# liaojing/videomorphing

Measured on AMD Instinct MI355X. Metric: Mpixel*iters/s (halfway optimizer, 1080p pair, 6-level pyramid, 500 iters/level), higher is better.
Workload: dtype f32

## Files before the change

include/vmorph.h:

```cpp
#ifndef VMORPH_H
#define VMORPH_H

#include <stdint.h>

#ifdef __cplusplus
extern "C" {
#endif

#define VM_OK            0
#define VM_E_INVALID    -1
#define VM_E_DEVICE     -2
#define VM_E_STATE      -3
#define VM_E_NUMERIC    -4
#define VM_E_CANCELLED  -5

typedef struct vm_ctx vm_ctx;
typedef struct vm_pyr vm_pyr;

enum { VM_BCOND_NONE = 0, VM_BCOND_CORNER = 1, VM_BCOND_BORDER = 2 };

typedef struct {
    float w_temp, w_ui, w_tps, w_ssim;
    float ssim_clamp;
    float eps;
// ... 29 lines not shown
    int    iters_live;
    double clk_shader_ticks[2];
    double clk_wall_ticks[2];
} vm_progress;

enum {
    VM_F_IMG0 = 0, VM_F_IMG1, VM_F_V, VM_F_LUMA, VM_F_MEAN, VM_F_VAR, VM_F_CROSS,
    VM_F_VALUE, VM_F_COUNTER, VM_F_TPS_AXY, VM_F_TPS_B, VM_F_UI_AXY, VM_F_UI_B,
    VM_F_IMPMASK,
    VM_F_TEMP_REF, VM_F_TEMP_MASK, VM_F_FLOW_F0, VM_F_FLOW_F1, VM_F_FLOW_B0, VM_F_FLOW_B1
};

const char *vm_last_error(void);
const char *vm_version(void);

int  vm_ctx_create(int device, vm_ctx **out);
void vm_ctx_destroy(vm_ctx *ctx);
int  vm_ctx_sync(vm_ctx *ctx);
int  vm_set_params(vm_ctx *ctx, const vm_kern_params *p);
int  vm_get_params(vm_ctx *ctx, vm_kern_params *p);
int  vm_set_math_mode(vm_ctx *ctx, int mode);
enum { VM_SWEEP_AUTO = 0, VM_SWEEP_TILE = 1, VM_SWEEP_SPLIT = 2, VM_SWEEP_STEP = 3, VM_SWEEP_SPARSE = 4, VM_SWEEP_PASS = 5 };
int  vm_set_tuning(vm_ctx *ctx, int sweep_mode, int threads, int parts);
int  vm_set_commit_order(vm_ctx *ctx, int order);
#define VM_REDUCE_ATOMIC 0
#define VM_REDUCE_ORDERED 1
int  vm_set_reduction(vm_ctx *ctx, int mode);
int  vm_dbg_pass_force_timeout(vm_ctx *ctx, int on);
int  vm_dbg_pass_fallbacks(vm_ctx *ctx);
int  vm_dbg_sparse_resident(vm_ctx *ctx, int mode);
int  vm_dbg_sparse_resident_visits(vm_ctx *ctx);
int  vm_dbg_pass_placement(vm_ctx *ctx, uint8_t *xcc_of_block, int n);
int  vm_dbg_golden(vm_ctx *ctx, int n, const float *params, float eps, uint32_t *out);
int  vm_dbg_streams_overlap(vm_ctx *a, vm_ctx *b, int *overlap);
int  vm_dbg_pyramid_scale(vm_ctx *ctx, const float *planes, int w, int h, int wout, int hout, float *out);
int  vm_device_info(vm_ctx *ctx, char *name256, int *cus, uint64_t *hbm_bytes);

int  vm_pyramid_create(vm_ctx *ctx, int nlevels, const int *w, const int *h, vm_pyr **out);
void vm_pyramid_destroy(vm_pyr *pyr);
int  vm_pyramid_levels(vm_pyr *pyr);
int  vm_level_dims(vm_pyr *pyr, int lvl, int *w, int *h, int *rowstride);
int  vm_level_upload_luma(vm_pyr *pyr, int lvl, const float *img0, const float *img1, int pitch);
int  vm_pyramid_build_rgb(vm_pyr *pyr, const uint8_t *rgb0, const uint8_t *rgb1, int pitch_bytes);
int  vm_level_set_v(vm_pyr *pyr, int lvl, const float *v_xy, int pitch);
int  vm_level_get_v(vm_pyr *pyr, int lvl, float *v_xy, int pitch);
int  vm_level_get_field(vm_pyr *pyr, int lvl, int field, void *host);
int  vm_level_clear(vm_pyr *pyr, int lvl);
int  vm_dbg_level_set_mask(vm_pyr *pyr, int lvl, const uint32_t *words);

int  vm_coarse_solve(vm_pyr *pyr, int lvl, int w0, int h0, const vm_constraint *c, int n);
int  vm_upsample_v(vm_pyr *pyr, int dst_lvl, int src_lvl);
int  vm_init_level(vm_pyr *pyr, int lvl, int w0, int h0, const vm_constraint *c, int n);
int  vm_optimize_level(vm_pyr *pyr, int lvl, float max_iter, volatile const int *run_flag,
                       int fixed_work, vm_progress *out);
int  vm_solve(vm_pyr *pyr, float max_iter, float max_iter_drop_factor,
              const vm_constraint *c, int n, volatile const int *run_flag,
              int fixed_work, vm_progress *per_level);
int  vm_optimize_level_batch(vm_pyr **pyrs, int n, int lvl, float max_iter,
                             volatile const int *run_flag, int fixed_work, vm_progress *out);
int  vm_solve_batch(vm_pyr **pyrs, int n, float max_iter, float max_iter_drop_factor,
                    volatile const int *run_flag, int fixed_work, vm_progress *per_level);
int  vm_solve_batch_cons(vm_pyr **pyrs, int n, float max_iter, float max_iter_drop_factor,
                         const vm_constraint *const *cons, const int *ncons,
                         volatile const int *run_flag, int fixed_work, vm_progress *per_level);
int  vm_upscale_result(vm_pyr *pyr, int lvl, int w0, int h0, float *v_xy_out, int pitch);

// ... 241 lines not shown
```

videomorphing_amd/capi.py:

```python
import ctypes as C
import os

_HERE = os.path.dirname(os.path.abspath(__file__))
LIB_PATH = os.environ.get("VM_LIB_PATH") or os.path.join(_HERE, "lib", "libvmorph_hip.so")

VM_OK = 0
VM_E_INVALID, VM_E_DEVICE, VM_E_STATE, VM_E_NUMERIC, VM_E_CANCELLED = -1, -2, -3, -4, -5
BCOND_NONE, BCOND_CORNER, BCOND_BORDER = 0, 1, 2
MATH_EXACT, MATH_FAST, MATH_EXACT_FMA, MATH_REF_FASTMATH, MATH_REF_TEX8, MATH_REF_TEX8_TRUNC = 0, 1, 2, 3, 4, 5
REDUCE_ATOMIC, REDUCE_ORDERED = 0, 1
DBG_MGB_QPATH = 3
SWEEP_AUTO, SWEEP_TILE, SWEEP_SPLIT, SWEEP_STEP, SWEEP_SPARSE, SWEEP_PASS = 0, 1, 2, 3, 4, 5
ERR_SSIM, ERR_TPS, ERR_UI, ERR_TEMP, ERR_ALL = 0, 1, 2, 3, 4
ERR_NAMES = ("ssim", "tps", "ui", "temp", "all")
EASE_LINEAR, EASE_SMOOTH = 0, 1
FILTER_BILINEAR, FILTER_CATMULL_ROM, FILTER_MITCHELL, FILTER_BSPLINE = 0, 1, 2, 3

FIELDS = {
    "img0": (0, 1), "img1": (1, 1), "v": (2, 2), "luma": (3, 2), "mean": (4, 2), "var": (5, 2),
    "cross": (6, 1), "value": (7, 1), "counter": (8, 1), "tps_axy": (9, 1), "tps_b": (10, 2),
    "ui_axy": (11, 1), "ui_b": (12, 2), "impmask": (13, 1),
    "temp_ref": (14, 2), "temp_mask": (15, 1), "f0": (16, 2), "f1": (17, 2), "b0": (18, 2), "b1": (19, 2),
}

SYMBOLS = [
    "vm_last_error", "vm_version", "vm_ctx_create", "vm_ctx_destroy", "vm_ctx_sync",
    "vm_set_params", "vm_get_params", "vm_set_math_mode", "vm_set_tuning", "vm_set_commit_order", "vm_set_reduction", "vm_dbg_pass_placement", "vm_dbg_pass_force_timeout",
    "vm_dbg_pass_fallbacks", "vm_dbg_golden", "vm_dbg_level_set_mask", "vm_dbg_sparse_resident", "vm_dbg_sparse_resident_visits", "vm_dbg_streams_overlap", "vm_dbg_pyramid_scale", "vm_device_info",
    "vm_pyramid_create", "vm_pyramid_destroy", "vm_pyramid_levels", "vm_level_dims",
    "vm_level_upload_luma", "vm_pyramid_build_rgb", "vm_level_set_v", "vm_level_get_v", "vm_level_get_field",
    "vm_level_clear", "vm_coarse_solve", "vm_upsample_v", "vm_init_level", "vm_optimize_level",
    "vm_solve", "vm_optimize_level_batch", "vm_solve_batch", "vm_solve_batch_cons", "vm_upscale_result", "vm_frame_create", "vm_frame_destroy", "vm_frame_upload", "vm_frame_upload_rgb",
    "vm_frame_download_ext", "vm_host_register", "vm_host_unregister", "vm_frame_set_v_from_level", "vm_render_halfway",
    "vm_render_halfway_dev", "vm_poisson_extend", "vm_poisson_extend_frames", "vm_frame_quadratic_path", "vm_frame_download_qpath", "vm_frame_download_v",
    "vm_rccl_bcast", "vm_rccl_comm_init_all", "vm_rccl_comm_destroy", "vm_bcast_params", "vm_bcast_bytes", "vm_dbg_poisson_profile",
    "vm_dbg_mgb_setup", "vm_dbg_mgb_level", "vm_dbg_mgb_cycle",
    "vm_video_create", "vm_video_destroy", "vm_video_levels", "vm_video_level_dims", "vm_video_upload_luma",
    "vm_video_upload_flows", "vm_video_build_rgb", "vm_video_build_flows", "vm_video_set_v", "vm_video_get_v",
    "vm_video_get_field", "vm_video_coarse_solve", "vm_video_upsample", "vm_video_init_level",
    "vm_video_initialize_temp", "vm_video_optimize_level", "vm_video_solve", "vm_video_result", "vm_frame_set_v_from_video",
    "vm_sync_level_table", "vm_sync_create", "vm_sync_destroy", "vm_sync_set_constraints", "vm_sync_load_identity",
    "vm_sync_upsample_level", "vm_sync_optimize_level", "vm_sync_solve", "vm_sync_get_field", "vm_sync_set_field",
    "vm_sync_result", "vm_sync_upload_frame", "vm_sync_upload_flow", "vm_sync_render", "vm_sync_render_dev",
    "vm_flow_params_default", "vm_optical_flow_rgb", "vm_optical_flow_luma", "vm_video_build_flows_rgb", "vm_sync_compute_flows",
    "vm_track_create", "vm_track_destroy", "vm_track_upload_frame", "vm_track_upload_flows", "vm_track_compute_flows",
    "vm_track_get_flows", "vm_track_propagate", "vm_video_build_flows_track",
    "vm_level_energy", "vm_level_energy_batch", "vm_level_error_map", "vm_level_error_image",
    "vm_video_energy", "vm_video_error_map", "vm_video_error_image",
    "vm_frame_sampling_maps", "vm_frame_upload_layers", "vm_render_layers", "vm_render_layers_dev",
    "vm_frame_upload_schedule", "vm_frame_clear_schedule", "vm_render_transition", "vm_render_transition_dev",
    "vm_render_transition_layers", "vm_render_transition_layers_dev", "vm_frame_transition_maps",
    "vm_render_shutter", "vm_render_shutter_dev", "vm_render_shutter_layers", "vm_render_shutter_layers_dev",
    "vm_render_transition_shutter", "vm_render_transition_shutter_dev", "vm_render_transition_shutter_layers",
    "vm_render_transition_shutter_layers_dev",
    "vm_render_viewport", "vm_render_viewport_dev", "vm_render_viewport_layers", "vm_render_viewport_layers_dev",
    "vm_frame_render_viewport_filtered", "vm_frame_render_viewport_filtered_dev", "vm_frame_render_viewport_filtered_layers",
    "vm_frame_render_viewport_filtered_layers_dev",
    "vm_render_viewport_shutter", "vm_render_viewport_shutter_dev", "vm_render_viewport_shutter_layers",
    "vm_render_viewport_shutter_layers_dev",
    "vm_render_viewport_transition_shutter", "vm_render_viewport_transition_shutter_dev",
    "vm_render_viewport_transition_shutter_layers", "vm_render_viewport_transition_shutter_layers_dev",
# ... 63 lines not shown
class VmError(RuntimeError):
    def __init__(self, code, msg):
        RuntimeError.__init__(self, "vmorph error %d: %s" % (code, msg))
        self.code = code


_lib = None


def load():
    global _lib
    if _lib is not None:
        return _lib
    if not os.path.exists(LIB_PATH):
        raise ImportError("%s is missing: run `python -m videomorphing_amd.build` "
                          "(or __graft_entry__.build()); there is no fallback path" % LIB_PATH)
    L = C.CDLL(LIB_PATH)
    vp, i, f = C.c_void_p, C.c_int, C.c_float
    L.vm_last_error.restype = C.c_char_p
    L.vm_version.restype = C.c_char_p
    sig = {
        "vm_ctx_create": [i, C.POINTER(vp)],
        "vm_ctx_sync": [vp],
        "vm_set_params": [vp, C.POINTER(KernParams)],
        "vm_get_params": [vp, C.POINTER(KernParams)],
        "vm_set_math_mode": [vp, i],
        "vm_set_tuning": [vp, i, i, i],
        "vm_set_commit_order": [vp, i],
        "vm_set_reduction": [vp, i],
        "vm_dbg_pass_placement": [vp, vp, i],
        "vm_dbg_pass_force_timeout": [vp, i],
        "vm_dbg_pass_fallbacks": [vp],
        "vm_dbg_golden": [vp, i, vp, C.c_float, vp],
        "vm_dbg_sparse_resident": [vp, C.c_int],
        "vm_dbg_sparse_resident_visits": [vp],
        "vm_device_info": [vp, C.c_char_p, C.POINTER(i), C.POINTER(C.c_uint64)],
        "vm_pyramid_create": [vp, i, C.POINTER(i), C.POINTER(i), C.POINTER(vp)],
        "vm_pyramid_levels": [vp],
        "vm_level_dims": [vp, i, C.POINTER(i), C.POINTER(i), C.POINTER(i)],
        "vm_level_upload_luma": [vp, i, vp, vp, i],
        "vm_pyramid_build_rgb": [vp, vp, vp, i],
        "vm_level_set_v": [vp, i, vp, i],
        "vm_level_get_v": [vp, i, vp, i],
        "vm_level_get_field": [vp, i, i, vp],
        "vm_level_clear": [vp, i],
        "vm_dbg_level_set_mask": [vp, i, vp],
        "vm_coarse_solve": [vp, i, i, i, vp, i],
        "vm_upsample_v": [vp, i, i],
        "vm_init_level": [vp, i, i, i, vp, i],
        "vm_optimize_level": [vp, i, f, vp, i, C.POINTER(Progress)],
        "vm_solve": [vp, f, f, vp, i, vp, i, vp],
        "vm_optimize_level_batch": [vp, i, i, f, vp, i, vp],
        "vm_solve_batch": [vp, i, f, f, vp, i, vp],
        "vm_solve_batch_cons": [vp, i, f, f, vp, vp, vp, i, vp],
        "vm_upscale_result": [vp, i, i, i, vp, i],
        "vm_frame_create": [vp, i, i, i, C.POINTER(vp)],
        "vm_frame_upload": [vp, vp, vp, vp, vp],
        "vm_frame_upload_rgb": [vp, vp, vp, i],
        "vm_dbg_streams_overlap": [vp, vp, C.POINTER(i)],
        "vm_dbg_pyramid_scale": [vp, vp, i, i, i, i, vp],
        "vm_frame_download_ext": [vp, i, vp],
        "vm_frame_set_v_from_level": [vp, vp, i],
        "vm_render_halfway": [vp, f, f, i, vp, i],
        "vm_render_halfway_dev": [vp, f, f, i, C.POINTER(f)],
        "vm_poisson_extend": [vp, i, f, i, C.POINTER(i), C.POINTER(f), C.POINTER(f)],
        "vm_poisson_extend_frames": [C.POINTER(vp), i, f, i, C.POINTER(i), C.POINTER(f), C.POINTER(f)],
# ... 126 lines not shown
```

videomorphing_amd/csrc/vm_api.cpp:

```cpp
#include "vm_internal.h"
#include "vm_host.h"

#include <algorithm>
#include <cstdarg>
#include <cstdio>
#include <cstdlib>
#include <cstring>
#include <string>
#include <vector>

static thread_local std::string g_err;

int vm_fail(int code, const char *fmt, ...)
{
    char buf[512];
    va_list ap;
    va_start(ap, fmt);
    vsnprintf(buf, sizeof(buf), fmt, ap);
    va_end(ap);
    g_err = buf;
    return code;
}

extern "C" const char *vm_last_error(void) { return g_err.c_str(); }
// ... 217 lines not shown
        memset(xcc_of_block, 0xFF, (size_t)n);
        return VM_OK;
    }
    std::vector<uint32_t> h(2048);
    VM_HIP(hipStreamSynchronize(c->stream));
    VM_HIP(hipMemcpy(h.data(), c->pass_dbg.get(), 2048 * sizeof(uint32_t), hipMemcpyDeviceToHost));
    for (int k = 0; k < n; ++k) xcc_of_block[k] = (uint8_t)(h[k] & 0xFFu);
    return VM_OK;
}

extern "C" int vm_dbg_golden(vm_ctx *c, int n, const float *params, float eps, uint32_t *out)
{
    if (!params || !out || n < 1 || n > 65536) return vm_fail(VM_E_INVALID, "vm_dbg_golden: bad argument");
    if (!(eps >= 1.0f / 1024.0f && eps <= 1.0f)) return vm_fail(VM_E_INVALID, "vm_dbg_golden: eps %g (2^-10 to 1)", (double)eps);
    for (int k = 0; k < n; ++k)
        if (!(params[4 * k] >= 0.0f && params[4 * k] <= 16.0f))
            return vm_fail(VM_E_INVALID, "vm_dbg_golden: cc of case %d is %g (0 to 16)", k, (double)params[4 * k]);
    VM_ENTER_LOCKED(c);
    VmDev<float> in;
    VmDev<uint32_t> res;
    const size_t words = (size_t)n * VM_DBG_GOLDEN_WORDS;
    if (int rc = in.reserve((size_t)4 * n)) return rc;
    if (int rc = res.reserve(words)) return rc;
    hipStream_t s = c->stream;
    VM_HIP(hipMemcpyAsync(in.get(), params, (size_t)4 * n * sizeof(float), hipMemcpyHostToDevice, s));
    VM_HIP(hipMemsetAsync(res.get(), 0, words * sizeof(uint32_t), s));
    vm_launch_dbg_golden_fast(n, in.get(), eps, res.get(), s);
    VM_HIP(hipGetLastError());
    VM_HIP(hipMemcpyAsync(out, res.get(), words * sizeof(uint32_t), hipMemcpyDeviceToHost, s));
    VM_HIP(hipStreamSynchronize(s));
    return VM_OK;
}

extern "C" int vm_set_tuning(vm_ctx *c, int sweep_mode, int threads, int parts)
{
    if (!c || sweep_mode < VM_SWEEP_AUTO || sweep_mode > VM_SWEEP_PASS || threads < 0 || parts < 0 ||
        (threads && (threads % 64 || threads < 256 || threads > 1024)) || parts > 64)
        return vm_fail(VM_E_INVALID, "vm_set_tuning: bad argument");
    c->sweep_mode = sweep_mode;
    c->sweep_threads = threads;
    c->sweep_parts = parts;
    return VM_OK;
}

extern "C" int vm_device_info(vm_ctx *c, char *name256, int *cus, uint64_t *hbm)
{
    VM_ENTER(c);
    hipDeviceProp_t pr;
    VM_HIP(hipGetDeviceProperties(&pr, c->device));
    if (name256) snprintf(name256, 256, "%s (%s)", pr.name, pr.gcnArchName);
    if (cus) *cus = pr.multiProcessorCount;
    if (hbm) *hbm = (uint64_t)pr.totalGlobalMem;
    return VM_OK;
}

int vm_level_alloc(vm_ctx *c, vm_level &l, bool with_images)
{
    size_t n = (size_t)l.rs * l.h;
    size_t off = 0;
    size_t o_v = off; off += vm_align256(n * 8);
    size_t o_img0 = off, o_img1 = off, o_luma = off, o_mean = off, o_var = off, o_tpsb = off,
           o_uib = off, o_cross = off, o_value = off, o_uiaxy = off, o_imp = off;
    if (with_images) {
        o_img0 = off; off += vm_align256(n * 4);
        o_img1 = off; off += vm_align256(n * 4);
        o_luma = off; off += vm_align256(n * 8);
// ... 394 lines not shown
```

videomorphing_amd/csrc/vm_internal.h:

```cpp
#ifndef VM_INTERNAL_H
#define VM_INTERNAL_H

#include <hip/hip_runtime.h>
#include <stdint.h>
#include "../../include/vmorph.h"

#define VM_TILE_W 64
#define VM_TILE_H 16
#define VM_PITCH_X 69
#define VM_PITCH_Y 21
#define VM_HALO_W (VM_TILE_W + 4)
#define VM_HALO_H (VM_TILE_H + 4)
#define VM_NCELL (VM_HALO_W * VM_HALO_H)

struct VmLevelView {
    int w, h, rs;
    float inv_wh;
    int imp_rs, imp_rows;
    const float *img0, *img1;
    float2 *v, *luma, *mean, *var, *tps_b, *ui_b;
    float *cross, *value, *ui_axy;
    uint32_t *impmask;
    uint32_t *rec_tag;
    float4 *rec_a, *rec_b;
// ... 44 lines not shown
                                           uint32_t *stats, int iter_idx, int fixed_work,     \
                                           int threads, int parts, hipStream_t s);            \
    void vm_launch_optimize_step_##SUFFIX(const VmLevelView *views, int nbatch, int cap, int w,  \
                                          int h, const VmKParams &P, const uint32_t *tables,  \
                                          int offx, int offy, int pi, int pj, uint32_t epoch, \
                                          uint32_t prev_epoch, int src, int decide,           \
                                          uint32_t *flags, uint32_t *stats, int iter_idx,     \
                                          int fixed_work, int threads, int parts,             \
                                          uint32_t *slots_cur, const uint32_t *slots_prev,    \
                                          int prev_iter_idx, hipStream_t s);                  \
    void vm_launch_optimize_pass_##SUFFIX(const VmLevelView *views, int nbatch, int cap, int w,  \
                                          int h, const VmKParams &P, const uint32_t *tables,  \
                                          int offx, int offy, uint32_t epoch0, uint32_t *bar, \
                                          uint32_t *flags, uint32_t *stats, int iter_idx,     \
                                          int fixed_work, uint32_t *slots_cur,                \
                                          const uint32_t *slots_prev, int prev_iter_idx,      \
                                          uint32_t *err, uint32_t *dbg, int decide,           \
                                          int force_wt, hipStream_t s);                       \
    int vm_pass_resident_blocks_##SUFFIX(int device);                                         \
    void vm_launch_upsample_##SUFFIX(float2 *dst, int dw, int dh, int drs, const float2 *src, \
                                     int sw, int sh, int srs, hipStream_t s);                 \
    void vm_launch_splat_##SUFFIX(const VmLevelView &L, int w0, int h0,                       \
                                  const vm_constraint *dev_c, int n, hipStream_t s);

VM_DECL_LAUNCHERS(exact)
VM_DECL_LAUNCHERS(fast)
VM_DECL_LAUNCHERS(exactf)
VM_DECL_LAUNCHERS(reffm)
VM_DECL_LAUNCHERS(tex8)
VM_DECL_LAUNCHERS(tex8t)

#define VM_DBG_GOLDEN_WORDS 20
void vm_launch_dbg_golden_fast(int n, const float *in, float eps, uint32_t *out, hipStream_t s);

void vm_launch_upscale(float2 *dst, int w0, int h0, int dpitch, const float2 *v, int w, int h,
                       int rs, hipStream_t s);
void vm_launch_blend_v(float2 *dst, int dpitch, const float2 *a, const float2 *b, int spitch, int w0, int h0,
                       float alpha, float beta, hipStream_t s);
void vm_launch_render(uint8_t *out, int out_pitch, int w, int h, int rs, int ex, float color_fa,
                      float geo_fa, int color_from, const uchar4 *ext0, const uchar4 *ext1,
                      const float2 *v, const float2 *u, hipStream_t s);

#endif
```

videomorphing_amd/csrc/vm_sweep_kernels.hip:

```cpp
#include <algorithm>
#include <type_traits>
#include "vm_morph_common.h"

typedef __attribute__((address_space(1))) const uint32_t vm_g_cu32;
typedef __attribute__((address_space(1))) uint32_t vm_g_u32;
typedef __attribute__((address_space(1))) const unsigned long long vm_g_cu64;
typedef __attribute__((address_space(1))) unsigned long long vm_g_u64;
typedef __attribute__((address_space(1))) const float vm_g_cf32;

__device__ __forceinline__ int mad24(int a, int b, int c) { return __mul24(a, b) + c; }

namespace {

__device__ __forceinline__ int tile_cols(int w) { return (w + VM_PITCH_X - 1) / VM_PITCH_X; }
__device__ __forceinline__ int tile_rows(int h) { return (h + VM_PITCH_Y - 1) / VM_PITCH_Y; }
__device__ __forceinline__ int tile_ox(int t, int gx, int offx) { return (t % gx) * VM_PITCH_X + offx; }
__device__ __forceinline__ int tile_oy(int t, int gx, int offy) { return (t / gx) * VM_PITCH_Y + offy; }
__device__ __forceinline__ int phase_px(int ox, int slot, int pj) { return ox + (slot & 31) * 2 + pj; }
__device__ __forceinline__ int phase_py(int oy, int slot, int pi) { return oy + (slot >> 5) * 2 + pi; }
__device__ __forceinline__ void stage_imp(uint32_t *imp, const uint32_t *tables, int tid, int T) { for (int k = tid; k < 225; k += T) imp[k] = tables[VM_TAB_IMP + k]; }
__device__ __forceinline__ void stage_tps(float *tps, const uint32_t *tables, int tid, int T) { for (int k = tid; k < 625; k += T) tps[k] = __uint_as_float(tables[VM_TAB_TPS + k]); }
__device__ __forceinline__ float cell_count(int qy, int h, int qx, int w) { return (float)(window_count(qy, h) * window_count(qx, w)); }
__device__ __forceinline__ int window_row(int k) { return (k * 13) >> 6; }

// ... 691 lines not shown
    fj = __builtin_amdgcn_fmed3f(fj, -1.0f, (float)L.h);
    const int i = clamp0(L.w - 1, (int)fi + t.cx), j = clamp0(L.h - 1, (int)fj + t.cy);
    wgt = fmaf(t.wxs, a, t.wxo) * fmaf(t.wys, b, t.wyo);
    return (uint32_t)(t.imgoff + j * L.rs + i) << 2;
}
__device__ __forceinline__ void taps32_issue(const VmLevelView &L, const TapLane &t, const PixelCtx &c, float vx,
                                             float vy, float &texel, float &wgt)
{
    texel = *(vm_g_cf32 *)((const char *)L.img0 + taps32_addr(L, t, c, vx, vy, wgt));
}
struct TexelKeep {
    uint32_t off = 0xFFFFFFFFu;
    float texel = 0.0f;
};
__device__ __forceinline__ void taps32_issue(const VmLevelView &L, const TapLane &t, const PixelCtx &c, float vx,
                                             float vy, TexelKeep &keep, float &texel, float &wgt)
{
    const uint32_t off = taps32_addr(L, t, c, vx, vy, wgt);
    if (off != keep.off) {
        keep.texel = *(vm_g_cf32 *)((const char *)L.img0 + off);
        keep.off = off;
    }
    texel = keep.texel;
}
__device__ __forceinline__ void taps32_finish(const TapLane &t, float texel, float wgt, float &lx, float &ly)
{
    float r = texel * wgt;
    r += dpp_xor1(r);
    r += dpp_xor2(r);
    const float o = dpp_half_mirror(r);
    lx = t.odd ? o : r;
    ly = t.odd ? r : o;
}
__device__ __forceinline__ void taps32(const VmLevelView &L, const TapLane &t, const PixelCtx &c, float vx, float vy,
                                       TexelKeep &keep, float &lx, float &ly)
{
    float texel, wgt;
    taps32_issue(L, t, c, vx, vy, keep, texel, wgt);
    taps32_finish(t, texel, wgt, lx, ly);
}
__device__ __forceinline__ void line_lumas(const VmLevelView &L, const TapLane &t, const PixelCtx &c, float gx, float gy,
                                           float tmin, TexelKeep &keep, float2 &luma)
{
    taps32(L, t, c, fmaf(gx, tmin, c.v.x), fmaf(gy, tmin, c.v.y), keep, luma.x, luma.y);
}

template <bool INTERIOR>
__device__ __forceinline__ float change32(const VmKParams &P, const Nb1 &nb, const PixelCtx &c, float lx, float ly)
{
    const float dmx = lx - c.old_luma.x, dmy = ly - c.old_luma.y;
    const float dvx = lx * lx - c.old_luma.x * c.old_luma.x;
    const float dvy = ly * ly - c.old_luma.y * c.old_luma.y;
    const float dcross = lx * ly - c.old_luma.x * c.old_luma.y;
    float acc;
    if (INTERIOR) {
        const float val = ssim_core(window_mean(nb.A, dmx, 0.04f), window_mean(nb.B, dmy, 0.04f), nb.VX + dvx, nb.VY + dvy,
                                    nb.X + dcross, 25.0f, P.ssim_clamp);
        acc = nb.N != 0.0f ? nb.VAL - val : 0.0f;
    } else {
        const bool valid = nb.N != 0.0f;
        const float n = valid ? nb.N : 25.0f;
        const float in = n == 25.0f ? 0.04f : __builtin_amdgcn_rcpf(n);
        const float val = ssim_core(window_mean(nb.A, dmx, in), window_mean(nb.B, dmy, in), nb.VX + dvx, nb.VY + dvy,
                                    nb.X + dcross, n, P.ssim_clamp);
        acc = valid ? nb.VAL - val : 0.0f;
    }
// ... 89 lines not shown
    }
    const float R = 0.618033989f, C = 1.0f - R;
    float a = 0;
    float b = cc * C, x = b * R + cc * C;
    float fb, fx;
    ELINE(b, fb);
    ELINE(x, fx);
#pragma unroll 1
    for (;;) {
        if (!(cc - a > P.eps))
            break;
        const bool lt = fx < fb;
        const float p = lt ? x : b, qv = lt ? cc : a;
        a = lt ? b : a;
        cc = lt ? cc : x;
        const float xn = p * R + qv * C;
        float f;
        ELINE(xn, f);
        const float ob = b, ofb = fb;
        b = lt ? x : xn;
        x = lt ? xn : ob;
        fb = lt ? fx : f;
        fx = lt ? f : ofb;
    }
#undef ELINE
    const float tmin = fx < fb ? x : b, fmin = fx < fb ? fx : fb;
    if (!(fmin < 0))
        return false;
    step = make_float2(gx * tmin, gy * tmin);
    line_lumas(L, tl, c, gx, gy, tmin, keep, luma);
    return true;
}

#define GOLDEN64_NO_TRACE(T_)
#define GOLDEN64(EVAL2_, TRACE_, CC_, EPS_, HI_, NEVAL_, TMIN_, FMIN_)                                                 \
    {                                                                                                                  \
        const float R = 0.618033989f, C = 1.0f - R;                                                                    \
        float a = 0;                                                                                                   \
        float b = (CC_) * C, x = b * R + (CC_) * C;                                                                    \
        float fb, fx;                                                                                                  \
        EVAL2_((HI_) ? x : b, fb, fx);                                                                                 \
        TRACE_(b)                                                                                                      \
        TRACE_(x)                                                                                                      \
        (NEVAL_) += 2;                                                                                                 \
        _Pragma("unroll 1") while ((CC_) > (EPS_) && !(fx < fb))                                                       \
        {                                                                                                              \
            const float xn = b * R, xn2 = xn * R;                                                                      \
            float f1, f2;                                                                                              \
            EVAL2_((HI_) ? xn2 : xn, f1, f2);                                                                          \
            TRACE_(xn)                                                                                                 \
              \
            const bool held = x > (EPS_) && !(fb < f1);                                                                \
            if (held) {                       \
                TRACE_(xn2)                                                                                            \
            }                                                                                                          \
            (NEVAL_) += held ? 2 : 1;                                                                                  \
            (CC_) = held ? b : x;                                                                                      \
            x = held ? xn : b;                                                                                         \
            b = held ? xn2 : xn;                                                                                       \
            fx = held ? f1 : fb;                                                                                       \
            fb = held ? f2 : f1;                                                                                       \
        }                                                                                                              \
        _Pragma("unroll 1") for (;;)                                                                                   \
        {                                                                                                              \
            if (!((CC_) - a > (EPS_)))                                                                                 \
                break;                                                                                                 \
            const bool lt = fx < fb;                                                                                   \
                          \
            const float p = lt ? x : b, qv = lt ? (CC_) : a;                                                           \
            const float a1 = lt ? b : a, cc1 = lt ? (CC_) : x;                                                         \
            const float xn = p * R + qv * C;                                                                           \
            const float b1 = lt ? x : xn, x1 = lt ? xn : b;                                                            \
             \
               \
                      \
                                                                               \
            const bool G = lt;                                                                                         \
            const float p2 = G ? x1 : b1, q2 = G ? cc1 : a1;                                                           \
            const float xn2 = p2 * R + q2 * C;                                                                         \
            float f1, f2;                                                                                              \
            EVAL2_((HI_) ? xn2 : xn, f1, f2);                                                                          \
            TRACE_(xn)                                                                                                 \
            ++(NEVAL_);                                                                                                \
            {                                                                                                          \
                const float nfb = lt ? fx : f1, nfx = lt ? f1 : fb;                                                    \
                a = a1;                                                                                                \
                (CC_) = cc1;                                                                                           \
                b = b1;                                                                                                \
                x = x1;                                                                                                \
                fb = nfb;                                                                                              \
                fx = nfx;                                                                                              \
            }                                                                                                          \
            if ((CC_) - a > (EPS_) && (fx < fb) == G) {          \
                TRACE_(xn2)                                                                                            \
                const float ob = b, ofb = fb;                                                                          \
                a = G ? b : a;                                                                                         \
                (CC_) = G ? (CC_) : x;                                                                                 \
                b = G ? x : xn2;                                                                                       \
                x = G ? xn2 : ob;                                                                                      \
                fb = G ? fx : f2;                                                                                      \
                fx = G ? f2 : ofb;                                                                                     \
                ++(NEVAL_);                                                                                            \
            }                                                                                                          \
        }                                                                                                              \
        (TMIN_) = fx < fb ? x : b;                                                                                     \
        (FMIN_) = fx < fb ? fx : fb;                                                                                   \
    }

template <bool INTERIOR, class Ring>
__device__ __forceinline__ bool decide64(const VmLevelView &L, const VmKParams &P, const Nb1 &nb, const Ring &ring,
                                         const PixelCtx &c, int sub, bool hi, float2 &step, float2 &luma,
                                         uint32_t &n_eval)
{
    n_eval += 4;
    const bool has_temp = L.temp_mask != nullptr;
    const float WT = has_temp ? P.w_temp * c.tmask * L.factor_d * L.inv_wh : 0.0f;
    const TapLane tl = tap_lane_make(L, sub);
    float lx, ly;
    float gx = 0, gy = 0;
    {
        const float sgn = hi ? -1.0f : 1.0f;
        float g_tex[2], g_wgt[2];
#pragma unroll
        for (int r = 0; r < 2; ++r) {
            const float dx = r == 0 ? sgn * P.eps : 0.0f, dy = r == 0 ? 0.0f : sgn * P.eps;
            taps32_issue(L, tl, c, c.v.x + dx, c.v.y + dy, g_tex[r], g_wgt[r]);
        }
#pragma unroll
        for (int r = 0; r < 2; ++r) {
            const float dx = r == 0 ? sgn * P.eps : 0.0f, dy = r == 0 ? 0.0f : sgn * P.eps;
            taps32_finish(tl, g_tex[r], g_wgt[r], lx, ly);
            const float change = change32<INTERIOR>(P, nb, c, lx, ly);
            const float dd = dx * dx + dy * dy;
            const float v_tps = fmaf(c.tps_axy, dd, fmaf(c.tps_b.x, dx, c.tps_b.y * dy));
            const float v_ui = fmaf(c.ui_axy, dd, fmaf(c.ui_b.x, dx, c.ui_b.y * dy));
            float e = (P.w_ui * v_ui + P.w_ssim * change) * L.inv_wh + P.w_tps * v_tps;
            if (has_temp)
                e = fmaf(WT, temp_change(c, dx, dy), e);
            e *= sgn;
            float e_lo, e_hi;
            halves(e, e_lo, e_hi);
            if (r == 0) {
                gx += e_lo;
                gx += e_hi;
            } else {
                gy += e_lo;
                gy += e_hi;
            }
        }
    }
    gx = -gx;
    gy = -gy;
    const float ng = fsqrt(gx * gx + gy * gy);
    if (ng == 0)
        return false;
    gx = fdiv(gx, ng);
    gy = fdiv(gy, ng);
    float cc = fmaxf(fover32(L, ring, c, gx, gy, sub) - P.eps, 0.0f);
    const float gg = gx * gx + gy * gy;
    const float WS = P.w_ssim * L.inv_wh, WU = P.w_ui * L.inv_wh;
    const float Q2 = (WU * c.ui_axy + P.w_tps * c.tps_axy) * gg;
    const float Q1 = WU * (c.ui_b.x * gx + c.ui_b.y * gy) + P.w_tps * (c.tps_b.x * gx + c.tps_b.y * gy);
    const float T0 = fabsf(c.v.x - c.tref.x) + fabsf(c.v.y - c.tref.y);
    TexelKeep keep;
#define ELINE2(T_, FLO_, FHI_)                                                         \
    {                                                                                  \
        const float nvx_ = fmaf(gx, (T_), c.v.x), nvy_ = fmaf(gy, (T_), c.v.y);        \
        taps32(L, tl, c, nvx_, nvy_, keep, lx, ly);                                    \
        float f_ = fmaf(WS, change32<INTERIOR>(P, nb, c, lx, ly), (T_) * fmaf(Q2, (T_), Q1)); \
        if (has_temp)                                                                  \
            f_ = fmaf(WT, (fabsf(nvx_ - c.tref.x) + fabsf(nvy_ - c.tref.y)) - T0, f_); \
        halves(f_, (FLO_), (FHI_));                                                    \
    }
    float tmin, fmin;
    GOLDEN64(ELINE2, GOLDEN64_NO_TRACE, cc, P.eps, hi, n_eval, tmin, fmin)
#undef ELINE2
    if (!(fmin < 0))
        return false;
    step = make_float2(gx * tmin, gy * tmin);
    line_lumas(L, tl, c, gx, gy, tmin, keep, luma);
    return true;
}
#endif

__device__ __forceinline__ void ctx_load(PixelCtx &c, const VmLevelView &L, const float *s_tps, int px, int py)
{
    c.px = px;
    c.py = py;
    c.idx = py * L.rs + px;
    c.v = L.v[c.idx];
    c.old_luma = L.luma[c.idx];
    c.ui_axy = L.ui_axy[c.idx];
    c.ui_b = L.ui_b[c.idx];
    c.tps_axy = s_tps[(border_class(py, L.h) * 5 + border_class(px, L.w)) * 25 + 12] / 2;
    c.tref = make_float2(0, 0);
    c.tmask = 0.0f;
    if (L.temp_mask) {
        c.tref = L.temp_ref[c.idx];
        c.tmask = L.temp_mask[c.idx];
    }
}

__device__ __forceinline__ bool is_interior(const VmLevelView &L, int px, int py)
{
    return px >= 4 && px < L.w - 4 && py >= 4 && py < L.h - 4;
}

struct MaskGeom {
    int bx0, by0, nbx, nby;
// ... 282 lines not shown
                    hit = true;
                    cand = !pixel_locked(L, P.bcond, px, py);
                }
                S.d_ok[tid] = state;
            }
            bool any_hit;
            const int n_act = compact256(cand, tid, S.list, S.wave_cnt, hit, &any_hit);
            if (!any_hit)
                continue;

            if (n_act > 0) {
                st_cand += n_act;
#if !VM_EXACT
                if (!DENSE || (SMAX > 7 && INTV && n_act * 32 <= T)) {
                    const bool wide = n_act * 64 <= T;
                    for (int base = 0; base < n_act; base += wide ? T / 64 : T / 32) {
                    const int li = base + (wide ? tid >> 6 : tid >> 5), sub = tid & 31;
                    const bool writer = wide ? (tid & 63) == 0 : sub == 0;
                    const int slot = S.list[min(li, n_act - 1)];
                    const int tx = slot & 31, ty = slot >> 5;
                    const int px = ox + tx * 2 + pj, py = oy + ty * 2 + pi;
                    const bool wave_interior = __all(li >= n_act || is_interior(L, px, py));
                    if (li < n_act) {
                        PixelCtx c;
                        ctx_load(c, L, S.tps, px, py);
                        LdsSrc src{&S, (ty * 2 + pi) * VM_HALO_W + (tx * 2 + pj)};
                        c.tps_b = S.tpsb[src.hc + 2 * VM_HALO_W + 2];
                        float2 step = make_float2(0, 0), luma = make_float2(0, 0);
                        Nb1 nb;
                        bool ok;
                        uint32_t n_eval = 0;
                        if (wave_interior) {
                            nb1_load<true>(nb, L, src, c, sub);
                            ok = wide ? decide64<true>(L, P, nb, RingGlobal{L.v}, c, sub, (tid & 32) != 0, step, luma, n_eval)
                                      : decide32<true>(L, P, nb, RingGlobal{L.v}, c, sub, step, luma, n_eval);
                        } else {
                            nb1_load<false>(nb, L, src, c, sub);
                            ok = wide ? decide64<false>(L, P, nb, RingGlobal{L.v}, c, sub, (tid & 32) != 0, step, luma, n_eval)
                                      : decide32<false>(L, P, nb, RingGlobal{L.v}, c, sub, step, luma, n_eval);
                        }
                        if (writer)
                            atomicAdd(&S.n_eval, n_eval);
                        if (ok && writer) {
                            S.d_step[slot] = step;
                            S.d_mean[slot] = commit_dmean(luma, c.old_luma);
                            S.d_var[slot] = commit_dvar(luma, c.old_luma);
                            S.d_cross[slot] = commit_dcross(luma.x, luma.y, c.old_luma.x, c.old_luma.y);
                            L.luma[c.idx] = luma;
                            L.ui_b[c.idx] = commit_ui_b(c.ui_b, c.ui_axy, step);
                            L.v[c.idx] = commit_v(c.v, step);
                            S.d_ok[slot] = 3;
                        }
                    }
                    }
                } else
#else
                if (n_act * 32 <= 4 * T) {
                    const bool wide = n_act * 64 <= T;
                    for (int base = 0; base < n_act; base += wide ? T / 64 : T / 32) {
                        const int li = base + (wide ? tid >> 6 : tid >> 5), sub = tid & 31;
                        const bool writer = wide ? (tid & 63) == 0 : sub == 0;
                        const int slot = S.list[min(li, n_act - 1)];
                        const int tx = slot & 31, ty = slot >> 5;
                        const int px = ox + tx * 2 + pj, py = oy + ty * 2 + pi;
                        if (li < n_act) {
                            PixelCtx c;
                            ctx_load(c, L, S.tps, px, py);
                            LdsSrc src{&S, (ty * 2 + pi) * VM_HALO_W + (tx * 2 + pj)};
                            c.tps_b = S.tpsb[src.hc + 2 * VM_HALO_W + 2];
                            float2 step;
                            uint32_t n_eval = 0;
// ... 2140 lines not shown
                                                        int prev_iter_idx, int nslot_prev, int ntiles, int ngroups, int cap, int spread)
{
    pass_sum_slots(stats, slots_prev, prev_iter_idx, nslot_prev, ntiles, ngroups, cap, (int)threadIdx.x, spread != 0);
}

__global__ void SUF(k_next_iter)(int *iter_dev, int set, int value)
{
    if (threadIdx.x == 0 && blockIdx.x == 0)
        *iter_dev = set ? value : *iter_dev + value;
}

#if !VM_EXACT
__global__ __launch_bounds__(64) void SUF(k_dbg_golden)(const float *__restrict__ in, float eps, uint32_t *__restrict__ out)
{
    const int k = (int)blockIdx.x;
    const bool hi = (threadIdx.x & 32) != 0;
    float cc = in[4 * k];
    const float A = in[4 * k + 1], t0 = in[4 * k + 2], B = in[4 * k + 3];
    uint32_t *o = out + (size_t)k * VM_DBG_GOLDEN_WORDS;
    uint32_t n_eval = 0;
    int n_pt = 0;
#define EGOLDEN(T_, FLO_, FHI_)                     \
    {                                               \
        const float d_ = (T_) - t0;                 \
        const float f_ = (A * d_) * d_ + B;         \
        halves(f_, (FLO_), (FHI_));                 \
    }
#define TGOLDEN(T_)                                             \
    {                                                           \
        if (threadIdx.x == 0 && n_pt < VM_DBG_GOLDEN_WORDS - 3) \
            o[3 + n_pt] = __float_as_uint(T_);                  \
        ++n_pt;                                                 \
    }
    float tmin, fmin;
    GOLDEN64(EGOLDEN, TGOLDEN, cc, eps, hi, n_eval, tmin, fmin)
#undef EGOLDEN
#undef TGOLDEN
    if (threadIdx.x == 0) {
        o[0] = __float_as_uint(tmin);
        o[1] = __float_as_uint(fmin);
        o[2] = n_eval;
    }
}
#endif

}

void SUF(vm_launch_optimize)(const VmLevelView *views, int nbatch, int cap, int w, int h, const VmKParams &P,
                             const uint32_t *tables, int offx, int offy, uint32_t *flags, uint32_t *stats,
                             int iter_idx, int fixed_work, int threads, const int *iter_dev, int dense,
                             uint32_t *tile_list, hipStream_t s)
{
    dim3 b(threads), g((w + VM_PITCH_X - 1) / VM_PITCH_X, (h + VM_PITCH_Y - 1) / VM_PITCH_Y, nbatch);
#if !VM_EXACT
    if (!dense && tile_list) {
        const int nwords = ((w + 4) / 5 + 2) * ((h + 4) / 5 + 2), tiles = (int)(g.x * g.y);
        hipLaunchKernelGGL(SUF(k_tile_scan), dim3(std::min((nwords + 255) / 256, 32), 1, nbatch), dim3(256), 0, s, views, cap, offx,
                           offy, flags, iter_idx, fixed_work, iter_dev, tile_list, tiles);
        hipLaunchKernelGGL(SUF(k_optimize_listed), dim3(std::min(tiles * nbatch, VM_TILE_LIST_GRID)), b, 0, s, views, cap, P, tables,
                           offx, offy, flags, stats, iter_idx, iter_dev, tile_list, tiles, nbatch);
        return;
    }
    if (!dense) {
        hipLaunchKernelGGL(SUF(k_optimize)<false>, g, b, 0, s, views, cap, P, tables, offx, offy, flags, stats,
                           iter_idx, fixed_work, iter_dev);
        return;
    }
    if (dense == 2) {
        hipLaunchKernelGGL((SUF(k_optimize)<true, 7, 4>), g, b, 0, s, views, cap, P, tables, offx, offy, flags, stats,
                           iter_idx, fixed_work, iter_dev);
        return;
    }
    if (dense == 3) {
        hipLaunchKernelGGL((SUF(k_optimize)<true, VM_SMAX, VM_MIN_FANOUT, false>), g, b, 0, s, views, cap, P, tables, offx, offy,
                           flags, stats, iter_idx, fixed_work, iter_dev);
// ... 70 lines not shown
                                  const uint32_t *slots_prev, int prev_iter_idx, uint32_t *err, uint32_t *dbg,
                                  int decide, int force_wt, hipStream_t s)
{
    const int gx = (w + VM_PITCH_X - 1) / VM_PITCH_X, gy = (h + VM_PITCH_Y - 1) / VM_PITCH_Y;
    const int ntiles = gx * gy, ngroups = ntiles * nbatch;
    const int nblocks = (ngroups + 7) / 8 * 256;
    if (!decide) {
        hipLaunchKernelGGL(SUF(k_pass_tail), dim3(1), dim3(64), 0, s, stats, slots_prev, prev_iter_idx, nblocks, ntiles, ngroups, cap,
                           force_wt & 4);
        return;
    }
    hipLaunchKernelGGL(SUF(k_pass), dim3(nblocks), dim3(VM_PASS_T), 0, s, views, cap, P, tables, offx, offy, epoch0, ngroups,
                       ntiles, bar, flags, stats, iter_idx, fixed_work, slots_cur, slots_prev, prev_iter_idx, nblocks, err,
                       dbg, force_wt);
}

int SUF(vm_pass_resident_blocks)(int device)
{
    hipDeviceProp_t pr;
    int per_cu = 0;
    if (hipGetDeviceProperties(&pr, device) != hipSuccess ||
        hipOccupancyMaxActiveBlocksPerMultiprocessor(&per_cu, SUF(k_pass), VM_PASS_T, 0) != hipSuccess) {
        (void)hipGetLastError();
        return 0;
    }
    return per_cu * pr.multiProcessorCount;
}

#if !VM_EXACT
void vm_launch_dbg_golden_fast(int n, const float *in, float eps, uint32_t *out, hipStream_t s)
{
    hipLaunchKernelGGL(SUF(k_dbg_golden), dim3(n), dim3(64), 0, s, in, eps, out);
}
#endif
```

Baseline: 1985.

## Batch golden-section tap fetches into a lane ladder via ds_swizzle

Measured after the change: 2026 (median of 6 runs). 2.1% higher.

```diff
diff --git a/include/vmorph.h b/include/vmorph.h
--- a/include/vmorph.h
+++ b/include/vmorph.h
@@ -85,6 +85,8 @@
 int  vm_dbg_sparse_resident_visits(vm_ctx *ctx);
 int  vm_dbg_pass_placement(vm_ctx *ctx, uint8_t *xcc_of_block, int n);
 int  vm_dbg_golden(vm_ctx *ctx, int n, const float *params, float eps, uint32_t *out);
+int  vm_dbg_ladder(vm_ctx *ctx, int w, int h, const float *img0, const float *img1, int n, const float *params,
+                   float eps, uint32_t *out);
 int  vm_dbg_streams_overlap(vm_ctx *a, vm_ctx *b, int *overlap);
 int  vm_dbg_pyramid_scale(vm_ctx *ctx, const float *planes, int w, int h, int wout, int hout, float *out);
 int  vm_device_info(vm_ctx *ctx, char *name256, int *cus, uint64_t *hbm_bytes);
diff --git a/videomorphing_amd/capi.py b/videomorphing_amd/capi.py
--- a/videomorphing_amd/capi.py
+++ b/videomorphing_amd/capi.py
@@ -26,7 +26,7 @@
 SYMBOLS = [
     "vm_last_error", "vm_version", "vm_ctx_create", "vm_ctx_destroy", "vm_ctx_sync",
     "vm_set_params", "vm_get_params", "vm_set_math_mode", "vm_set_tuning", "vm_set_commit_order", "vm_set_reduction", "vm_dbg_pass_placement", "vm_dbg_pass_force_timeout",
-    "vm_dbg_pass_fallbacks", "vm_dbg_golden", "vm_dbg_level_set_mask", "vm_dbg_sparse_resident", "vm_dbg_sparse_resident_visits", "vm_dbg_streams_overlap", "vm_dbg_pyramid_scale", "vm_device_info",
+    "vm_dbg_pass_fallbacks", "vm_dbg_golden", "vm_dbg_ladder", "vm_dbg_level_set_mask", "vm_dbg_sparse_resident", "vm_dbg_sparse_resident_visits", "vm_dbg_streams_overlap", "vm_dbg_pyramid_scale", "vm_device_info",
     "vm_pyramid_create", "vm_pyramid_destroy", "vm_pyramid_levels", "vm_level_dims",
     "vm_level_upload_luma", "vm_pyramid_build_rgb", "vm_level_set_v", "vm_level_get_v", "vm_level_get_field",
     "vm_level_clear", "vm_coarse_solve", "vm_upsample_v", "vm_init_level", "vm_optimize_level",
@@ -156,6 +156,7 @@
         "vm_dbg_pass_force_timeout": [vp, i],
         "vm_dbg_pass_fallbacks": [vp],
         "vm_dbg_golden": [vp, i, vp, C.c_float, vp],
+        "vm_dbg_ladder": [vp, i, i, vp, vp, i, vp, C.c_float, vp],
         "vm_dbg_sparse_resident": [vp, C.c_int],
         "vm_dbg_sparse_resident_visits": [vp],
         "vm_device_info": [vp, C.c_char_p, C.POINTER(i), C.POINTER(C.c_uint64)],
diff --git a/videomorphing_amd/csrc/vm_api.cpp b/videomorphing_amd/csrc/vm_api.cpp
--- a/videomorphing_amd/csrc/vm_api.cpp
+++ b/videomorphing_amd/csrc/vm_api.cpp
@@ -273,6 +273,37 @@
     return VM_OK;
 }
 
+extern "C" int vm_dbg_ladder(vm_ctx *c, int w, int h, const float *img0, const float *img1, int n, const float *params,
+                             float eps, uint32_t *out)
+{
+    if (!img0 || !img1 || !params || !out || n < 1 || n > 65536 || w < 2 || h < 2 || w > 64 || h > 64)
+        return vm_fail(VM_E_INVALID, "vm_dbg_ladder: bad argument");
+    if (!(eps >= 1.0f / 1024.0f && eps <= 1.0f)) return vm_fail(VM_E_INVALID, "vm_dbg_ladder: eps %g (2^-10 to 1)", (double)eps);
+    for (int k = 0; k < n; ++k) {
+        const float *q = params + 8 * k;
+        if (!(q[0] >= 0.0f && q[0] <= (float)(w - 1) && q[1] >= 0.0f && q[1] <= (float)(h - 1)))
+            return vm_fail(VM_E_INVALID, "vm_dbg_ladder: pixel of case %d is (%g, %g)", k, (double)q[0], (double)q[1]);
+        if (!(q[6] >= 0.0f && q[6] <= 16.0f)) return vm_fail(VM_E_INVALID, "vm_dbg_ladder: cc of case %d is %g (0 to 16)", k, (double)q[6]);
+    }
+    VM_ENTER_LOCKED(c);
+    VmDev<float> img, in;
+    VmDev<uint32_t> res;
+    const size_t px = (size_t)w * h, words = (size_t)n * VM_DBG_LADDER_WORDS;
+    if (int rc = img.reserve(2 * px)) return rc;
+    if (int rc = in.reserve((size_t)8 * n)) return rc;
+    if (int rc = res.reserve(words)) return rc;
+    hipStream_t s = c->stream;
+    VM_HIP(hipMemcpyAsync(img.get(), img0, px * sizeof(float), hipMemcpyHostToDevice, s));
+    VM_HIP(hipMemcpyAsync(img.get() + px, img1, px * sizeof(float), hipMemcpyHostToDevice, s));
+    VM_HIP(hipMemcpyAsync(in.get(), params, (size_t)8 * n * sizeof(float), hipMemcpyHostToDevice, s));
+    VM_HIP(hipMemsetAsync(res.get(), 0, words * sizeof(uint32_t), s));
+    vm_launch_dbg_ladder_fast(img.get(), w, h, n, in.get(), eps, res.get(), s);
+    VM_HIP(hipGetLastError());
+    VM_HIP(hipMemcpyAsync(out, res.get(), words * sizeof(uint32_t), hipMemcpyDeviceToHost, s));
+    VM_HIP(hipStreamSynchronize(s));
+    return VM_OK;
+}
+
 extern "C" int vm_set_tuning(vm_ctx *c, int sweep_mode, int threads, int parts)
 {
     if (!c || sweep_mode < VM_SWEEP_AUTO || sweep_mode > VM_SWEEP_PASS || threads < 0 || parts < 0 ||
diff --git a/videomorphing_amd/csrc/vm_internal.h b/videomorphing_amd/csrc/vm_internal.h
--- a/videomorphing_amd/csrc/vm_internal.h
+++ b/videomorphing_amd/csrc/vm_internal.h
@@ -100,6 +100,9 @@
 
 #define VM_DBG_GOLDEN_WORDS 20
 void vm_launch_dbg_golden_fast(int n, const float *in, float eps, uint32_t *out, hipStream_t s);
+#define VM_DBG_LADDER_POINTS 40
+#define VM_DBG_LADDER_WORDS (1 + 5 * VM_DBG_LADDER_POINTS)
+void vm_launch_dbg_ladder_fast(const float *img, int w, int h, int n, const float *in, float eps, uint32_t *out, hipStream_t s);
 
 void vm_launch_upscale(float2 *dst, int w0, int h0, int dpitch, const float2 *v, int w, int h,
                        int rs, hipStream_t s);
diff --git a/videomorphing_amd/csrc/vm_sweep_kernels.hip b/videomorphing_amd/csrc/vm_sweep_kernels.hip
--- a/videomorphing_amd/csrc/vm_sweep_kernels.hip
+++ b/videomorphing_amd/csrc/vm_sweep_kernels.hip
@@ -747,6 +747,11 @@
     lx = t.odd ? o : r;
     ly = t.odd ? r : o;
 }
+template <int K>
+__device__ __forceinline__ float ladder_take(float x)
+{
+    return __int_as_float(__builtin_amdgcn_ds_swizzle(__float_as_int(x), 0x07 | (K << 8)));
+}
 __device__ __forceinline__ void taps32(const VmLevelView &L, const TapLane &t, const PixelCtx &c, float vx, float vy,
                                        TexelKeep &keep, float &lx, float &ly)
 {
@@ -902,34 +907,80 @@
     return true;
 }
 
+
+__device__ __forceinline__ float ladder_pick(bool hi, int oct, float l0, float h0, float l1, float h1, float l2, float h2,
+                                             float l3, float h3)
+{
+    const float p0 = hi ? h0 : l0, p1 = hi ? h1 : l1, p2 = hi ? h2 : l2, p3 = hi ? h3 : l3;
+    const float p01 = (oct & 1) ? p1 : p0, p23 = (oct & 1) ? p3 : p2;
+    return (oct & 2) ? p23 : p01;
+}
+#define LADDER_FETCH(K_, BLX_, BLY_, PLX_, PLY_, LX_, LY_)  \
+    {                                                       \
+        if ((K_) == 0) {                                    \
+            (LX_) = ladder_take<0>(BLX_);                   \
+            (LY_) = ladder_take<0>(BLY_);                   \
+        } else {                                            \
+            (LX_) = (PLX_);                                 \
+            (LY_) = (PLY_);                                 \
+        }                                                   \
+        if ((K_) != 3) {                                    \
+            (PLX_) = ladder_take<((K_) + 1) & 3>(BLX_);     \
+            (PLY_) = ladder_take<((K_) + 1) & 3>(BLY_);     \
+        }                                                   \
+    }
 #define GOLDEN64_NO_TRACE(T_)
-#define GOLDEN64(EVAL2_, TRACE_, CC_, EPS_, HI_, NEVAL_, TMIN_, FMIN_)                                                 \
+#define GOLDEN64_NO_BATCH(T_)
+#define GOLDEN64_REGIME_ROUND(EVALB_, TRACE_, K_, CC_, EPS_, HI_, NEVAL_)                                              \
+    {                                                                                                                  \
+        const float xn = b * R, xn2 = xn * R;                                                                          \
+        float f1, f2;                                                                                                  \
+        EVALB_(K_, (HI_) ? xn2 : xn, f1, f2);                                                                          \
+        TRACE_(xn)                                                                                                     \
+              \
+        const bool held = x > (EPS_) && !(fb < f1);                                                                    \
+        if (held) {                           \
+            TRACE_(xn2)                                                                                                \
+        }                                                                                                              \
+        (NEVAL_) += held ? 2 : 1;                                                                                      \
+        (CC_) = held ? b : x;                                                                                          \
+        x = held ? xn : b;                                                                                             \
+        b = held ? xn2 : xn;                                                                                           \
+        fx = held ? f1 : fb;                                                                                           \
+        fb = held ? f2 : f1;                                                                                           \
+    }
+#define GOLDEN64(EVAL2_, BATCH_, EVALB_, TRACE_, CC_, EPS_, HI_, OCT_, NEVAL_, TMIN_, FMIN_)                           \
     {                                                                                                                  \
         const float R = 0.618033989f, C = 1.0f - R;                                                                    \
         float a = 0;                                                                                                   \
         float b = (CC_) * C, x = b * R + (CC_) * C;                                                                    \
         float fb, fx;                                                                                                  \
-        EVAL2_((HI_) ? x : b, fb, fx);                                                                                 \
+        {                     \
+            const float q1 = b * R, q2 = q1 * R, q3 = q2 * R, q4 = q3 * R, q5 = q4 * R, q6 = q5 * R;                   \
+            BATCH_(ladder_pick((HI_), (OCT_), b, x, q1, q2, q3, q4, q5, q6))                                           \
+        }                                                                                                              \
+        EVALB_(0, (HI_) ? x : b, fb, fx);                                                                              \
         TRACE_(b)                                                                                                      \
         TRACE_(x)                                                                                                      \
         (NEVAL_) += 2;                                                                                                 \
-        _Pragma("unroll 1") while ((CC_) > (EPS_) && !(fx < fb))                                                       \
-        {                                                                                                              \
-            const float xn = b * R, xn2 = xn * R;                                                                      \
-            float f1, f2;                                                                                              \
-            EVAL2_((HI_) ? xn2 : xn, f1, f2);                                                                          \
-            TRACE_(xn)                                                                                                 \
-              \
-            const bool held = x > (EPS_) && !(fb < f1);                                                                \
-            if (held) {                       \
-                TRACE_(xn2)                                                                                            \
+        _Pragma("unroll 1") for (;;) {                                          \
+            if (!((CC_) > (EPS_) && !(fx < fb)))                                                                       \
+                break;                                                                                                 \
+            GOLDEN64_REGIME_ROUND(EVALB_, TRACE_, 1, CC_, EPS_, HI_, NEVAL_)                                           \
+            if (!((CC_) > (EPS_) && !(fx < fb)))                                                                       \
+                break;                                                                                                 \
+            GOLDEN64_REGIME_ROUND(EVALB_, TRACE_, 2, CC_, EPS_, HI_, NEVAL_)                                           \
+            if (!((CC_) > (EPS_) && !(fx < fb)))                                                                       \
+                break;                                                                                                 \
+            GOLDEN64_REGIME_ROUND(EVALB_, TRACE_, 3, CC_, EPS_, HI_, NEVAL_)                                           \
+            if (!((CC_) > (EPS_) && !(fx < fb)))                                                                       \
+                break;                                                                                                 \
+            {                       \
+                const float q1 = b * R, q2 = q1 * R, q3 = q2 * R, q4 = q3 * R, q5 = q4 * R, q6 = q5 * R, q7 = q6 * R,  \
+                            q8 = q7 * R;                                                                               \
+                BATCH_(ladder_pick((HI_), (OCT_), q1, q2, q3, q4, q5, q6, q7, q8))                                     \
             }                                                                                                          \
-            (NEVAL_) += held ? 2 : 1;                                                                                  \
-            (CC_) = held ? b : x;                                                                                      \
-            x = held ? xn : b;                                                                                         \
-            b = held ? xn2 : xn;                                                                                       \
-            fx = held ? f1 : fb;                                                                                       \
-            fb = held ? f2 : f1;                                                                                       \
+            GOLDEN64_REGIME_ROUND(EVALB_, TRACE_, 0, CC_, EPS_, HI_, NEVAL_)                                           \
         }                                                                                                              \
         _Pragma("unroll 1") for (;;)                                                                                   \
         {                                                                                                              \
@@ -977,7 +1028,7 @@
         (FMIN_) = fx < fb ? fx : fb;                                                                                   \
     }
 
-template <bool INTERIOR, class Ring>
+template <bool INTERIOR, bool LADDER = true, class Ring>
 __device__ __forceinline__ bool decide64(const VmLevelView &L, const VmKParams &P, const Nb1 &nb, const Ring &ring,
                                          const PixelCtx &c, int sub, bool hi, float2 &step, float2 &luma,
                                          uint32_t &n_eval)
@@ -1042,9 +1093,28 @@
             f_ = fmaf(WT, (fabsf(nvx_ - c.tref.x) + fabsf(nvy_ - c.tref.y)) - T0, f_); \
         halves(f_, (FLO_), (FHI_));                                                    \
     }
+    float blx, bly;
+    float plx, ply;
+#define LADDER2(T_)                                                                             \
+    if (LADDER)                                                                                 \
+        taps32(L, tl, c, fmaf(gx, (T_), c.v.x), fmaf(gy, (T_), c.v.y), keep, blx, bly);
+#define ELINE2B(K_, T_, FLO_, FHI_)                                                    \
+    {                                                                                  \
+        const float nvx_ = fmaf(gx, (T_), c.v.x), nvy_ = fmaf(gy, (T_), c.v.y);        \
+        if (LADDER)                                                                    \
+            LADDER_FETCH(K_, blx, bly, plx, ply, lx, ly)                               \
+        else                                                                           \
+            taps32(L, tl, c, nvx_, nvy_, keep, lx, ly);                                \
+        float f_ = fmaf(WS, change32<INTERIOR>(P, nb, c, lx, ly), (T_) * fmaf(Q2, (T_), Q1)); \
+        if (has_temp)                                                                  \
+            f_ = fmaf(WT, (fabsf(nvx_ - c.tref.x) + fabsf(nvy_ - c.tref.y)) - T0, f_); \
+        halves(f_, (FLO_), (FHI_));                                                    \
+    }
     float tmin, fmin;
-    GOLDEN64(ELINE2, GOLDEN64_NO_TRACE, cc, P.eps, hi, n_eval, tmin, fmin)
+    GOLDEN64(ELINE2, LADDER2, ELINE2B, GOLDEN64_NO_TRACE, cc, P.eps, hi, sub >> 3, n_eval, tmin, fmin)
 #undef ELINE2
+#undef ELINE2B
+#undef LADDER2
     if (!(fmin < 0))
         return false;
     step = make_float2(gx * tmin, gy * tmin);
@@ -1393,11 +1463,11 @@
                         uint32_t n_eval = 0;
                         if (wave_interior) {
                             nb1_load<true>(nb, L, src, c, sub);
-                            ok = wide ? decide64<true>(L, P, nb, RingGlobal{L.v}, c, sub, (tid & 32) != 0, step, luma, n_eval)
+                            ok = wide ? decide64<true, false>(L, P, nb, RingGlobal{L.v}, c, sub, (tid & 32) != 0, step, luma, n_eval)
                                       : decide32<true>(L, P, nb, RingGlobal{L.v}, c, sub, step, luma, n_eval);
                         } else {
                             nb1_load<false>(nb, L, src, c, sub);
-                            ok = wide ? decide64<false>(L, P, nb, RingGlobal{L.v}, c, sub, (tid & 32) != 0, step, luma, n_eval)
+                            ok = wide ? decide64<false, false>(L, P, nb, RingGlobal{L.v}, c, sub, (tid & 32) != 0, step, luma, n_eval)
                                       : decide32<false>(L, P, nb, RingGlobal{L.v}, c, sub, step, luma, n_eval);
                         }
                         if (writer)
@@ -3604,8 +3674,10 @@
             o[3 + n_pt] = __float_as_uint(T_);                  \
         ++n_pt;                                                 \
     }
+#define EGOLDENB(K_, T_, FLO_, FHI_) EGOLDEN(T_, FLO_, FHI_)
     float tmin, fmin;
-    GOLDEN64(EGOLDEN, TGOLDEN, cc, eps, hi, n_eval, tmin, fmin)
+    GOLDEN64(EGOLDEN, GOLDEN64_NO_BATCH, EGOLDENB, TGOLDEN, cc, eps, hi, 0, n_eval, tmin, fmin)
+#undef EGOLDENB
 #undef EGOLDEN
 #undef TGOLDEN
     if (threadIdx.x == 0) {
@@ -3613,6 +3685,72 @@
         o[1] = __float_as_uint(fmin);
         o[2] = n_eval;
     }
+}
+
+__global__ __launch_bounds__(64) void SUF(k_dbg_ladder)(const float *__restrict__ img, int w, int h, const float *__restrict__ in,
+                                                        float eps, uint32_t *__restrict__ out)
+{
+    const int k = (int)blockIdx.x;
+    const bool hi = (threadIdx.x & 32) != 0;
+    const int sub = (int)threadIdx.x & 31;
+    const float *q = in + 8 * k;
+    VmLevelView L = {};
+    L.w = w;
+    L.h = h;
+    L.rs = w;
+    L.img0 = img;
+    L.img1 = img + w * h;
+    PixelCtx c = {};
+    c.px = (int)q[0];
+    c.py = (int)q[1];
+    c.v = make_float2(q[2], q[3]);
+    const float gx = q[4], gy = q[5];
+    float cc = q[6];
+    uint32_t *o = out + (size_t)k * VM_DBG_LADDER_WORDS;
+    const TapLane tl = tap_lane_make(L, sub);
+    TexelKeep keep, keep_one;
+    float blx, bly, plx = 0.0f, ply = 0.0f;
+    uint32_t n_eval = 0;
+    int n_pt = 0;
+#define RLADDER(T_, LX_, LY_)                                                                                   \
+    {                                                                                                           \
+        float ox_, oy_;                                                                                         \
+        taps32(L, tl, c, fmaf(gx, (T_), c.v.x), fmaf(gy, (T_), c.v.y), keep_one, ox_, oy_);                     \
+        const int s_ = n_pt + (hi ? 1 : 0);                                                                     \
+        if (sub == 0 && s_ < VM_DBG_LADDER_POINTS) {                                                            \
+            o[1 + 5 * s_] = __float_as_uint(T_);                                                                \
+            o[2 + 5 * s_] = __float_as_uint(LX_);                                                               \
+            o[3 + 5 * s_] = __float_as_uint(LY_);                                                               \
+            o[4 + 5 * s_] = __float_as_uint(ox_);                                                               \
+            o[5 + 5 * s_] = __float_as_uint(oy_);                                                               \
+        }                                                                                                       \
+        n_pt += 2;                                                                                              \
+    }
+#define BLADDER(T_) taps32(L, tl, c, fmaf(gx, (T_), c.v.x), fmaf(gy, (T_), c.v.y), keep, blx, bly);
+#define ELADDERB(K_, T_, FLO_, FHI_)                     \
+    {                                                    \
+        float lx_, ly_;                                  \
+        LADDER_FETCH(K_, blx, bly, plx, ply, lx_, ly_)   \
+        RLADDER(T_, lx_, ly_)                            \
+        halves((T_), (FLO_), (FHI_));                    \
+    }
+#define ELADDER(T_, FLO_, FHI_)                                                              \
+    {                                                                                        \
+        float lx_, ly_;                                                                      \
+        taps32(L, tl, c, fmaf(gx, (T_), c.v.x), fmaf(gy, (T_), c.v.y), keep, lx_, ly_);      \
+        RLADDER(T_, lx_, ly_)                                                                \
+        halves((T_), (FLO_), (FHI_));                                                        \
+    }
+    float tmin, fmin;
+    GOLDEN64(ELADDER, BLADDER, ELADDERB, GOLDEN64_NO_TRACE, cc, eps, hi, sub >> 3, n_eval, tmin, fmin)
+#undef ELADDER
+#undef ELADDERB
+#undef BLADDER
+#undef RLADDER
+    (void)tmin;
+    (void)fmin;
+    if (threadIdx.x == 0)
+        o[0] = (uint32_t)n_pt;
 }
 #endif
 
@@ -3749,4 +3887,8 @@
 {
     hipLaunchKernelGGL(SUF(k_dbg_golden), dim3(n), dim3(64), 0, s, in, eps, out);
 }
+void vm_launch_dbg_ladder_fast(const float *img, int w, int h, int n, const float *in, float eps, uint32_t *out, hipStream_t s)
+{
+    hipLaunchKernelGGL(SUF(k_dbg_ladder), dim3(n), dim3(64), 0, s, img, w, h, in, eps, out);
+}
 #endif
```
